# takkasila/practical_path_guiding_lab

Hardware: AMD Instinct MI355X
Metric: Msamples/s guided, veach-ajar 1920x1080 max_depth 13 (higher is better)
Workload: dtype f32; 1 GPU; veach-ajar 1920x1080, max_depth 13, 16 one-sample training passes (main.py:192, 218) per step in one batched launch (the whole film), guided iteration 6 (SD-tree trained by rendering iterations 0-5, 252 spp); full PathGuidingIntegrator.sample(): camera rays, NEE, BSDF/SD-tree MIS, record list, po...; spp_per_pass=16, passes_per_launch=16, steps_per_launch=1, kd_leaves=21429, quad_records=1675769, jump_bits=6, kd_grid_bits=6, bytes_jump_tables=1404370944, pixels_per_rank_min=2073600, pixels_per_rank_max=2073600

## Files before the change

### practical_path_guiding_lab_amd/csrc/pg_kernels_splat.hip

```cpp
#include "pg_descent.hpp"
#include "pg_kernels.hpp"
#include "pg_splat_dev.hpp"

namespace pg {

constexpr int kBlock = 256;
static_assert(kBlock == kStageThreads, "stage_kd_planes copies one plane per thread");

__device__ __forceinline__ void plan_record(const TreeView &t, const AccumView &a, const uint4 *s_kd, int store_nee,
                                            float x, float y, float z, float dx, float dy, float radiance,
                                            float wo_pdf, float nx, float ny, float nee_lum, SlotAdd &path,
                                            SlotAdd &nee, unsigned &kd_lv, unsigned &q_lv, unsigned &q_q, unsigned &bytes)
{
	const bool inside = inside_root(t, x, y, z);
	KdNode leaf;
	uint32_t lv;
	kd_descend_grid(t, reinterpret_cast<const float *>(s_kd), x, y, z, inside, leaf, lv);
	kd_lv += stat_levels(lv);
	bytes += stat_bytes(lv);
	const uint32_t tree = leaf.tree;
	const TreeHead head = load_head_s(t.head, tree);
	const JumpPre pre_p = jump_prefetch(t.jump, tree, dx, dy, in_unit_square(dx, dy));
	const JumpPre pre_n = jump_prefetch(t.jump, tree, nx, ny, store_nee != 0 && in_unit_square(nx, ny));
	const float w = wo_pdf > 0.0f ? radiance / wo_pdf : 0.0f;
// ... 121 lines not shown
	const bool single = t.n_rec == 0 && t.n_trees == 1;
	long long v[4] = {0, 0, 0, 0};
	unsigned kd_lv = 0, q_lv = 0, q_q = 0, did = 0, st_bytes = 0;
	for (uint64_t base = (uint64_t)blockIdx.x * kBlock; base < total; base += (uint64_t)gridDim.x * kBlock) {
		const uint64_t g = base + threadIdx.x;
		float radiance = 0.0f, nee_lum = 0.0f, wp = 0.0f;
		SlotAdd path = {nullptr, 0, 0, 0, 0}, nee = {nullptr, 0, 0, 0, 0};
		bool keep = false;
		if (g < total) keep = process_slot(g, S, num_rays, g / (uint64_t)max_depth, r.active[g] != 0, l_final, r, radiance, nee_lum, wp);
		if (keep) {
			plan_record(t, a, s_kd, store_nee, r.position[g], r.position[S + g], r.position[2 * S + g], r.direction[g],
			            r.direction[S + g], radiance, wp, r.direction_nee[g], r.direction_nee[S + g], nee_lum, path, nee,
			            kd_lv, q_lv, q_q, st_bytes);
			++did;
		}
		if (single) {
			if (path.ptr) { v[0] += path.w0; v[1] += path.w1; v[2] += path.w2; v[3] += path.w3; }
			if (nee.ptr) { v[0] += nee.w0; v[1] += nee.w1; v[2] += nee.w2; v[3] += nee.w3; }
		} else {
			coop_add(path, s_val, s_ptr);
			if (store_nee) coop_add(nee, s_val, s_ptr);
		}
	}
	if (single) {
		__syncthreads();
#pragma unroll
		for (int k = 0; k < 4; ++k) {
			const unsigned long long sw = wave_sum_s((unsigned long long)v[k]);
			if ((threadIdx.x & 63) == 0) s_val[(threadIdx.x >> 6) * 4 + k] = (long long)sw;
		}
		__syncthreads();
		if (threadIdx.x < 4) {
			unsigned long long tot = 0;
			for (int w = 0; w < kBlock / 64; ++w) tot += (unsigned long long)s_val[w * 4 + threadIdx.x];
			if (tot) atomicAdd(reinterpret_cast<unsigned long long *>(a.root_acc + threadIdx.x), tot);
		}
	}
	count_depths_s(dc, kd_lv, did, q_lv, q_q, st_bytes);
}

__global__ __launch_bounds__(kBlock) void k_splat_list(TreeView t, AccumView a, int store_nee, uint64_t num_rays,
                                                       int32_t max_depth, const float *__restrict__ l_final,
                                                       const uint4 *__restrict__ l_final_q, pg_list_records r,
                                                       const uint32_t *__restrict__ live_count)
{
	__shared__ long long s_val[kBlock * 4];
	__shared__ unsigned long long s_ptr[kBlock];
	const uint64_t S = num_rays * (uint64_t)max_depth;
	uint64_t total = num_rays;
	for (int b = 0; b + 1 < max_depth; ++b) total += live_count[b];
	if ((uint64_t)blockIdx.x * kBlock >= total) return;
	const bool single = t.n_rec == 0 && t.n_trees == 1;
	long long v[4] = {0, 0, 0, 0};
	for (uint64_t base = (uint64_t)blockIdx.x * kBlock; base < total; base += (uint64_t)gridDim.x * kBlock) {
		const uint64_t g = base + threadIdx.x;
		SlotAdd path = {nullptr, 0, 0, 0, 0}, nee = {nullptr, 0, 0, 0, 0};
		if (g < total) {
#define PG_LD(p) __builtin_nontemporal_load(p)
			const uint32_t ray = PG_LD(r.ray_of + g);
			if (ray != kNoRay) {
				float in[3], lf[3];
				if (l_final_q) {
					const uint4 q = l_final_q[ray];
					lf[0] = __uint_as_float(q.x); lf[1] = __uint_as_float(q.y); lf[2] = __uint_as_float(q.z);
				} else {
					lf[0] = l_final[ray]; lf[1] = l_final[num_rays + ray]; lf[2] = l_final[2 * num_rays + ray];
				}
#pragma unroll
				for (int ch = 0; ch < 3; ++ch) {
					float out = (lf[ch] - PG_LD(r.throughput_radiance + ch * S + g)) / PG_LD(r.throughput_bsdf + ch * S + g);
					if (out != out) out = 0.0f;
					float q = out / PG_LD(r.bsdf + ch * S + g);
					if (q != q) q = 0.0f;
					in[ch] = q;
				}
				float radiance = luminance(in[0], in[1], in[2]);
				if (radiance != radiance) radiance = 0.0f;
				const float nee_lum = PG_LD(r.nee_lum + g);
				const float wp = PG_LD(r.wo_pdf + g);
				const bool both_zero = (radiance == 0.0f) && (nee_lum == 0.0f);
				if (!both_zero && !(wp == 0.0f) && !(wp != wp)) {
					const uint2 sl = r.slot[g];
					const uint32_t tf = PG_LD(r.tree + g), tree = tf & 0x7fffffffu;
#undef PG_LD
					const bool inside = (tf >> 31) != 0u;
					const float w = wp > 0.0f ? radiance / wp : 0.0f;
					const float wn = wp > 0.0f ? nee_lum / wp : 0.0f;
					if (sl.x != kSlotNone) {
						const Limbs q = quantize_weight(w);
						path.ptr = sl.x == kSlotRoot ? a.root_acc + (size_t)kAccWords * tree : a.rec_acc + (size_t)kAccWords * sl.x;
						path.w0 = q.l0; path.w1 = q.l1; path.w2 = q.l2; path.w3 = inside ? 1 : 0;
					} else if (inside) {
						atomicAdd(a.leaf_count + tree, 1ull);
					}
					if (store_nee && sl.y != kSlotNone) {
						const Limbs q = quantize_weight(wn);
						nee.ptr = sl.y == kSlotRoot ? a.root_acc + (size_t)kAccWords * tree : a.rec_acc + (size_t)kAccWords * sl.y;
						nee.w0 = q.l0; nee.w1 = q.l1; nee.w2 = q.l2; nee.w3 = 0;
					}
				}
			}
		}
		if (single) {
			if (path.ptr) { v[0] += path.w0; v[1] += path.w1; v[2] += path.w2; v[3] += path.w3; }
			if (nee.ptr) { v[0] += nee.w0; v[1] += nee.w1; v[2] += nee.w2; v[3] += nee.w3; }
		} else {
			coop_add(path, s_val, s_ptr);
			if (store_nee) coop_add(nee, s_val, s_ptr);
		}
	}
	if (single) {
		__syncthreads();
#pragma unroll
		for (int k = 0; k < 4; ++k) {
			const unsigned long long sw = wave_sum_s((unsigned long long)v[k]);
			if ((threadIdx.x & 63) == 0) s_val[(threadIdx.x >> 6) * 4 + k] = (long long)sw;
		}
		__syncthreads();
		if (threadIdx.x < 4) {
			unsigned long long tot = 0;
			for (int w = 0; w < kBlock / 64; ++w) tot += (unsigned long long)s_val[w * 4 + threadIdx.x];
			if (tot) atomicAdd(reinterpret_cast<unsigned long long *>(a.root_acc + threadIdx.x), tot);
		}
	}
}

constexpr unsigned kSplatGroupsPerCu = 64;

static inline dim3 grid_for(uint64_t n) { return dim3((unsigned)((n + kBlock - 1) / kBlock)); }

void launch_splat(const TreeView &t, const AccumView &a, int store_nee, uint64_t m, const pg_records &rec,
                  const uint32_t *d_count, DepthCounters *dc, hipStream_t s)
{
	if (m == 0) return;
	hipLaunchKernelGGL(k_splat, grid_for(m), dim3(kBlock), 0, s, t, a, store_nee, m, rec.position,
	                   rec.direction, rec.radiance, rec.wo_pdf, rec.direction_nee, rec.radiance_nee_lum,
	                   d_count, dc);
}

void launch_process_records(uint64_t num_rays, int32_t max_depth, const float *l_final,
                            const pg_dense_records &rec, const pg_records_out &out, uint32_t *d_count,
                            hipStream_t s)
{
	const uint64_t S = num_rays * (uint64_t)max_depth;
	(void)hipMemsetAsync(d_count, 0, sizeof(uint32_t), s);
	if (S == 0) return;
	hipLaunchKernelGGL(k_process_records, grid_for(S), dim3(kBlock), 0, s, num_rays, max_depth, l_final, rec,
	                   out, d_count);
}

static dim3 strided_grid(uint64_t S)
{
	static int cus[64] = {0};
	int dev = 0;
	(void)hipGetDevice(&dev);
// ... 31 lines not shown
```

### practical_path_guiding_lab_amd/csrc/pg_render.hip

```cpp
#include "pg_render_dev.hpp"
#include "pg_scene_state.hpp"

namespace pg {


constexpr int kBounceStash = 17;
typedef __attribute__((address_space(3))) float LdsFloat;
template <bool kFirst, int kGeneral, bool kStash = false>
__device__ __forceinline__ bool bounce_lane(const RenderArgs &a, const uint4 *s_kd, const uint64_t lane,
                                            const uint64_t rec_slot, const uint32_t depth, LdsFloat *stash = nullptr)
{
	const uint64_t N = a.n_lanes;
	const int D = a.max_depth;
	const float f = a.frac;
	const Shapes &sh = a.shapes;
	Pcg32 rng;
	v3 ray_o, ray_d, thr, L, prev_p;
	float prev_bsdf_pdf;
	const bool prev_delta = kFirst;
	const float ior = 1.0f;
	static_assert(kGeneral < 2, "mesh scenes run the split pipeline of pg_render_wave.hip");
	if (kFirst) {
		const uint64_t pixel = global_pixel(a, lane / (uint64_t)a.spp);
		rng = lane_stream(a.seed, a.spp, a.batched, pixel, (uint32_t)(lane % (uint64_t)a.spp));
// ... 234 lines not shown
{
	__shared__ float s_planes[3 * kKdGridPlanes];
	const uint4 *s_kd = reinterpret_cast<const uint4 *>(s_planes);
	__shared__ uint32_t s_wave[kRBlock / 64];
	__shared__ uint32_t s_base;
	__shared__ float s_stash[kBounceStash][kRBlock];
	uint64_t tid;
	bool alive;
	if (!wave_entry<kFirst>(a, tid, alive)) return;
	if (a.guided || a.record) stage_kd_planes(s_planes, a.tree);
	const uint64_t lane = alive ? (kFirst ? tid : (uint64_t)a.order_in[tid]) : 0;
	const uint64_t rec_base = kFirst ? 0 : records_before(a);
	bool cont = false;
	if (alive) cont = bounce_lane<kFirst, kGeneral, true>(a, s_kd, lane, rec_base + tid, (uint32_t)a.bounce, (LdsFloat *)&s_stash[0][threadIdx.x]);
	if (a.last) return;
	const unsigned long long ballot = __ballot(cont);
	const unsigned wl = threadIdx.x & 63u, wv = threadIdx.x >> 6;
	if (wl == 0) s_wave[wv] = (uint32_t)__popcll(ballot);
	__syncthreads();
	if (threadIdx.x == 0) {
		uint32_t tot = 0;
		for (int w = 0; w < kRBlock / 64; ++w) tot += s_wave[w];
		s_base = tot ? atomicAdd(&a.live_count[a.bounce], tot) : 0u;
	}
	__syncthreads();
	if (cont) {
		uint32_t off = s_base + (uint32_t)__popcll(ballot & ((1ull << wl) - 1ull));
		for (unsigned w = 0; w < wv; ++w) off += s_wave[w];
		a.order_out[off] = (uint32_t)lane;
	}
}

template <int kGeneral>
__global__ __launch_bounds__(kRBlock) void k_bounce_tail(RenderArgs a)
{
	__shared__ float s_planes[3 * kKdGridPlanes];
	const uint4 *s_kd = reinterpret_cast<const uint4 *>(s_planes);
	const uint64_t tid = (uint64_t)blockIdx.x * kRBlock + threadIdx.x;
	const uint64_t live = (uint64_t)live_final(a, a.bounce - 1);
	if (live > kTailPaths || (uint64_t)blockIdx.x * kRBlock >= live) return;
	if (tail_took_over(a, a.bounce - 1)) return;
	if (a.guided || a.record) stage_kd_planes(s_planes, a.tree);
	bool alive = tid < live;
	const uint64_t lane = alive ? (uint64_t)a.order_in[tid] : 0;
	const uint64_t rec_base = records_before(a);
	const uint64_t tail_base = rec_base + live;
	uint64_t slot = rec_base + tid;
	for (int depth = a.bounce; depth < a.max_depth; ++depth) {
		if (alive) alive = bounce_lane<false, kGeneral>(a, s_kd, lane, slot, (uint32_t)depth);
		if (!tail_next_slot(a, depth, alive, tail_base, slot)) break;
	}
}

__global__ __launch_bounds__(kRBlock) void k_layout_L(const uint4 *__restrict__ Lq, float *__restrict__ L, uint64_t N)
{
	const uint64_t i = (uint64_t)blockIdx.x * kRBlock + threadIdx.x;
	if (i >= N) return;
	const uint4 q = Lq[i];
	L[i] = __uint_as_float(q.x); L[N + i] = __uint_as_float(q.y); L[2 * N + i] = __uint_as_float(q.z);
}

__global__ __launch_bounds__(kRBlock) void k_finish(RenderArgs a, uint8_t *__restrict__ valid_out,
                                                    float *__restrict__ sumL, float *__restrict__ sumL2)
{
	const uint64_t pix = (uint64_t)blockIdx.x * kRBlock + threadIdx.x;
	if (pix >= a.n_pixels) return;
	const uint64_t N = a.n_lanes, P = a.film_pixels;
	const uint64_t gpix = global_pixel(a, pix);
	const uint64_t first = pix * (uint64_t)a.spp;
	if (valid_out)
		for (int s = 0; s < a.spp; ++s) valid_out[first + s] = a.hit0[first + s];
	if (sumL && sumL2) {
		float s1[3], s2[3];
		for (int c = 0; c < 3; ++c) { s1[c] = sumL[c * P + gpix]; s2[c] = sumL2[c * P + gpix]; }
		for (int s = 0; s < a.spp; ++s)
			for (int c = 0; c < 3; ++c) {
				const float v = a.L[c * N + first + s];
				s1[c] = s1[c] + v;
				s2[c] = s2[c] + v * v;
			}
		for (int c = 0; c < 3; ++c) { sumL[c * P + gpix] = s1[c]; sumL2[c * P + gpix] = s2[c]; }
	}
}

__global__ __launch_bounds__(kRBlock) void k_math_eval(int which, uint64_t n, const float *__restrict__ x,
                                                       float *__restrict__ out)
{
	const uint64_t i = (uint64_t)blockIdx.x * kRBlock + threadIdx.x;
	if (i >= n) return;
	const float v = x[i];
	float r, c;
	switch (which) {
	case 0: r = exp_f32(v); break;
	case 1: r = log_f32(v); break;
	case 2: r = erf_f32(v); break;
	case 3: r = erfinv_f32(v); break;
	case 4: sincos_f32(v, r, c); break;
	default: sincos_f32(v, c, r); break;
	}
	out[i] = r;
}

__device__ __forceinline__ float tent1(float d)
{
	const float a = 1.0f - fabs_(d);
	return a > 0.0f ? a : 0.0f;
}

__device__ __forceinline__ float gauss1(float d)
{
	const float a = exp_f32(-2.0f * (d * d)) - exp_f32(-8.0f);
	return a > 0.0f ? a : 0.0f;
}

template <int kFilter, bool kBatched>
__global__ __launch_bounds__(kRBlock) void k_film(uint32_t seed, int spp, int W, int H,
                                                  const float *__restrict__ L, float *__restrict__ out,
                                                  uint32_t stripe_rows, uint32_t stripe_index, uint32_t stripe_count,
                                                  float *__restrict__ acc, float scale, int acc_set)
{
	constexpr int R = kFilter == 1 ? 2 : 1;
	const uint64_t npix = (uint64_t)W * (uint64_t)H, N = npix * (uint64_t)spp;
	const uint64_t o = (uint64_t)blockIdx.x * kRBlock + threadIdx.x;
	if (o >= npix) return;
	const int x = (int)(o % (uint64_t)W), y = (int)(o / (uint64_t)W);
	if (stripe_count > 1u && ((uint32_t)y / stripe_rows) % stripe_count != stripe_index) return;
	const float cx = (float)x + 0.5f, cy = (float)y + 0.5f;
	for (int img = 0; img < (kBatched ? spp : 1); ++img) {
		float a0 = 0.0f, a1 = 0.0f, a2 = 0.0f, wsum = 0.0f;
		for (int ny = y - R; ny <= y + R; ++ny)
			for (int nx = x - R; nx <= x + R; ++nx) {
				if (nx < 0 || ny < 0 || nx >= W || ny >= H) continue;
				const uint64_t pix = (uint64_t)ny * (uint64_t)W + (uint64_t)nx;
				for (int s = kBatched ? img : 0; s < (kBatched ? img + 1 : spp); ++s) {
					const uint64_t lane = pix * (uint64_t)spp + (uint64_t)s;
// ... 245 lines not shown
		                                     (ctx->filter_spatial ? "stochastic box" : "nearest") + ", directional " +
		                                     (ctx->filter_directional ? "box" : "nearest") + "); reset it to nearest / nearest, record through pg_splat / pg_process_and_splat, or set the scene with pg_render_record_geometry on");
	PG_HIP(ctx, hipSetDevice(ctx->device));
	const pg_camera &cam = ctx->render->scene.cam;
	const uint64_t film = (uint64_t)cam.width * (uint64_t)cam.height;
	if (prm->pixel_begin > film || prm->pixel_count > film - prm->pixel_begin)
		return fail(ctx, PG_ERR_INVALID, "pg_render_pass: pixel range outside the film");
	P = prm->pixel_count ? prm->pixel_count : film - prm->pixel_begin;
	if (prm->stripe_count > 1) {
		if (prm->stripe_rows == 0 || prm->stripe_index >= prm->stripe_count || prm->pixel_begin != 0)
			return fail(ctx, PG_ERR_INVALID, "pg_render_pass: bad stripe parameters");
		uint64_t rows = 0;
		for (uint64_t row = 0; row < (uint64_t)cam.height; ++row)
			rows += (row / prm->stripe_rows) % prm->stripe_count == prm->stripe_index;
		if (prm->pixel_count && prm->pixel_count != rows * (uint64_t)cam.width)
			return fail(ctx, PG_ERR_INVALID, "pg_render_pass: pixel_count does not match the stripes of this rank");
		P = rows * (uint64_t)cam.width;
	}
	if (P == 0) return PG_OK;
	if (P * (uint64_t)prm->spp * (uint64_t)ctx->max_depth > 0xffffffffull)
		return fail(ctx, PG_ERR_INVALID, "pg_render_pass: more than 2^32 record slots in one pass");
	if (prm->slot < 0 || prm->slot > 1) return fail(ctx, PG_ERR_INVALID, "pg_render_pass: slot must be 0 or 1");
	return PG_OK;
}

static RenderArgs pass_args(pg_context *ctx, const pg_pass_params *prm, PassBuf &b, uint64_t P, float *L_out)
{
	const pg_render_state *r = ctx->render;
	const int D = ctx->max_depth;
	RenderArgs a;
	a.tree = ctx->view();
	const SceneState &sc = r->scene;
	a.shapes.quads = sc.quads.p; a.shapes.spheres = sc.spheres.p; a.shapes.boxes = sc.boxes.p; a.shapes.tris = sc.tris.p;
	a.shapes.tri_normals = sc.have_tri_normals ? sc.tri_normals.p : nullptr;
	a.shapes.tri_uvs = sc.have_tri_uvs ? sc.tri_uvs.p : nullptr;
	a.shapes.textures = sc.textures.p; a.shapes.texels = sc.texels.p; a.shapes.srgb_lut = sc.srgb_lut.p;
	a.shapes.bvh = sc.bvh.p; a.shapes.n_bvh_nodes = sc.n_bvh_nodes;
	a.shapes.n_quads = sc.n_quads; a.shapes.n_spheres = sc.n_spheres; a.shapes.n_boxes = sc.n_boxes;
	a.mats = sc.mats.p; a.emitters = sc.emitters.p; a.n_emitters = sc.n_emitters; a.ior = r->ior.p;
	a.dir_lights.lights = sc.dir_lights.p;
	for (int c = 0; c < 4; ++c) a.dir_lights.bsphere[c] = sc.bsphere[c];
	a.cam = sc.cam;
	a.n_lanes = P * (uint64_t)prm->spp; a.n_pixels = P; a.pixel_begin = prm->pixel_begin;
	a.stripe_rows = prm->stripe_rows; a.stripe_index = prm->stripe_index; a.stripe_count = prm->stripe_count;
	a.film_pixels = (uint64_t)r->scene.cam.width * (uint64_t)r->scene.cam.height;
	a.spp = prm->spp; a.max_depth = D; a.rr_depth = prm->rr_depth; a.seed = prm->seed; a.batched = prm->batched ? 1 : 0;
	a.guided = ctx->iteration > 1 ? 1 : 0;
	a.record = ctx->is_final ? 0 : 1; a.store_nee = ctx->store_nee; a.frac = ctx->bsdf_fraction;
	a.dc = ctx->dc_on ? ctx->dc : nullptr;
	a.ph = ctx->ph_on ? ctx->ph_buf.p : nullptr;
	const bool wave = r->scene.general >= 2;
	a.fuse_guide = wave && r->stages < 2 && !(r->overlap & 1) ? 1 : 0;
	if (r->scene.geometry && a.record) a.fuse_guide = 0;
	a.ray_d = b.ray_d.p; a.thr = b.thr.p; a.L = L_out; a.prev_p = b.prev_p.p;
	a.prev_pdf = b.prev_pdf.p; a.prev_quad = b.prev_quad.p; a.hit0 = b.hit0.p;
	a.rng_state = b.rng_state.p; a.rng_inc = b.rng_inc.p; a.live_count = b.live_count.p;
	a.ray_of = b.ray_of.p; a.r_bsdf = b.r_bsdf.p; a.r_tb = b.r_tb.p;
	a.r_tr = b.r_tr.p; a.r_nee = b.r_nee.p; a.r_wp = b.r_wp.p;
	a.r_slot = b.r_slot.p; a.r_tree = b.r_tree.p;
	a.Lq = wave ? b.Lq.p : nullptr;
	a.ws = b.ws.p; a.bvh_ovf = b.bvh_ovf.p; a.shadow_list = b.shadow_list.p;
	a.cast_count = b.live_count.p + (D + 1);
	a.shadow_count = b.live_count.p + (D + 1) + 2 * D;
	a.st_in = nullptr; a.st_out = nullptr; a.inc_in = nullptr; a.inc_out = nullptr;
	a.sort_key = nullptr; a.perm = nullptr; a.carry_in = nullptr; a.carry_out = nullptr; a.n_sort = 0;
	return a;
}

static void quad_bounce(pg_render_state *r, const RenderArgs &a, int it, hipStream_t s)
{
	Timed t(r, s, Timer::Bounce);
	if (tail_checkpoint(it, a.max_depth)) {
		const dim3 tgrid((unsigned)((kTailPaths + kRBlock - 1) / kRBlock));
		if (r->scene.general == 1) hipLaunchKernelGGL((k_bounce_tail<1>), tgrid, dim3(kRBlock), 0, s, a);
		else hipLaunchKernelGGL((k_bounce_tail<0>), tgrid, dim3(kRBlock), 0, s, a);
	}
	const dim3 grid((unsigned)((a.n_lanes + kRBlock - 1) / kRBlock));
	if (r->scene.general == 1) {
		if (it == 0) hipLaunchKernelGGL((k_bounce<true, 1>), grid, dim3(kRBlock), 0, s, a);
		else hipLaunchKernelGGL((k_bounce<false, 1>), grid, dim3(kRBlock), 0, s, a);
	} else {
		if (it == 0) hipLaunchKernelGGL((k_bounce<true, 0>), grid, dim3(kRBlock), 0, s, a);
		else hipLaunchKernelGGL((k_bounce<false, 0>), grid, dim3(kRBlock), 0, s, a);
	}
}

static bool worth_sorting(const PassBuf &b, int bounce, int sort_until, uint64_t N)
{
	if (bounce < 1 || bounce >= sort_until) return false;
	return !b.live_known || (uint64_t)b.live_prev[bounce - 1] * kSortMinLiveDen >= N * kSortMinLiveNum;
}

static Timer timer_of(WaveStage stage)
{
	switch (stage) {
	case WaveStage::Trace: return Timer::Trace;
	case WaveStage::ShadeA: case WaveStage::Shade: return Timer::ShadeA;
	case WaveStage::Cast: return Timer::Shadow;
	case WaveStage::Guide: return Timer::Guide;
	case WaveStage::ShadeB: return Timer::ShadeB;
	case WaveStage::Tail: break;
	}
	return Timer::Tail;
}

static int wave_bounce(pg_context *ctx, PassBuf &b, RenderArgs &a, int it, int sort_until, hipStream_t s)
{
	pg_render_state *r = ctx->render;
	const uint64_t N = a.n_lanes;
	const unsigned blocks = (unsigned)((N + kRBlock - 1) / kRBlock);
	uint32_t *const geo = r->scene.geometry && a.record ? b.r_geo.p : nullptr;
	auto launch = [&](WaveStage stage, hipStream_t on, unsigned grid_blocks) {
		Timed t(r, on, timer_of(stage));
		launch_wave_stage(stage, r->scene.general, it == 0, a, grid_blocks, (unsigned)ctx->n_cus, on, geo);
	};
	a.st_in = b.st[it & 1].p; a.inc_in = b.inc[it & 1].p;
	a.st_out = b.st[(it + 1) & 1].p; a.inc_out = b.inc[(it + 1) & 1].p;
	const bool sorted = worth_sorting(b, it, sort_until, N);
	a.carry_in = sorted ? b.carry[it & 1].p : nullptr;
	a.sort_key = nullptr; a.perm = nullptr; a.carry_out = nullptr;
	if (tail_checkpoint(it, a.max_depth)) launch(WaveStage::Tail, s, (unsigned)((kTailPaths + kRBlock - 1) / kRBlock));
	a.sort_key = sorted ? b.sort_key.p : nullptr;
	a.carry_out = worth_sorting(b, it + 1, sort_until, N) ? b.carry[(it + 1) & 1].p : nullptr;
	const bool fork = (r->overlap & 1) && !sorted;
	if (fork && !b.side) {
		PG_HIP(ctx, hipStreamCreateWithFlags(&b.side, hipStreamNonBlocking));
		PG_HIP(ctx, hipEventCreateWithFlags(&b.ev_fork, hipEventDisableTiming));
		PG_HIP(ctx, hipEventCreateWithFlags(&b.ev_join, hipEventDisableTiming));
	}
	if (sorted) {
		const uint64_t n_sort = b.live_known ? (uint64_t)b.live_prev[it - 1] + (uint64_t)b.live_prev[it - 1] / 32 + 65536 : N;
		a.n_sort = (uint32_t)(n_sort < N ? n_sort : N);
		PG_HIP(ctx, hipMemsetAsync(b.sort_key.p, 0xff, (size_t)a.n_sort * sizeof(uint16_t), s));
	}
	launch(WaveStage::Trace, s, blocks);
	if (sorted) {
		Timed t(r, s, Timer::Sort);
		PG_HIP(ctx, sort_places16(b.sort_tmp.p, b.sort_tmp_bytes, b.sort_key.p, b.sort_key_out.p, b.sort_perm.p, a.n_sort,
		                            a.live_count + (it - 1), s));
		a.perm = b.sort_perm.p;
	}
	if (r->stages == 0 && !(r->overlap & 1) && !geo) {
		launch(WaveStage::Shade, s, blocks);
		return PG_OK;
	}
	launch(WaveStage::ShadeA, s, blocks);
	if (fork) {
		PG_HIP(ctx, hipEventRecord(b.ev_fork, s));
		PG_HIP(ctx, hipStreamWaitEvent(b.side, b.ev_fork, 0));
		launch(WaveStage::Guide, b.side, blocks);
		PG_HIP(ctx, hipEventRecord(b.ev_join, b.side));
	}
	launch(WaveStage::Cast, s, blocks);
	if (fork) PG_HIP(ctx, hipStreamWaitEvent(s, b.ev_join, 0));
	else if (!a.fuse_guide) launch(WaveStage::Guide, s, blocks);
	launch(WaveStage::ShadeB, s, blocks);
	return PG_OK;
}

static pg_list_geometry list_geometry(const PassBuf &b, uint64_t S)
{
	pg_list_geometry g;
	const float *f = reinterpret_cast<const float *>(b.r_geo.p);
	g.position = f + GEO_P * S; g.direction = f + GEO_WO * S; g.direction_nee = f + GEO_NEE * S;
	g.depth = b.r_geo.p + GEO_DEPTH * S;
	return g;
}

static pg_list_records list_records(const PassBuf &b)
{
	pg_list_records lr;
	lr.ray_of = b.ray_of.p; lr.bsdf = b.r_bsdf.p; lr.throughput_bsdf = b.r_tb.p; lr.throughput_radiance = b.r_tr.p;
	lr.nee_lum = b.r_nee.p; lr.wo_pdf = b.r_wp.p; lr.slot = b.r_slot.p; lr.tree = b.r_tree.p;
	return lr;
}

static int finish_pass(pg_context *ctx, int slot, const RenderArgs &a, uint8_t *valid_out, float *sumL, float *sumL2, hipStream_t s)
{
	pg_render_state *r = ctx->render;
	PassBuf &b = r->pb[slot];
	if (a.record) {
		Timed t(r, s, Timer::Splat);
		const pg_list_records lr = list_records(b);
		if (r->scene.geometry && ctx->filtered_launch())
			launch_splat_list_filtered(ctx->view(), ctx->f.accum_view(), ctx->filter_args(), ctx->store_nee, a.n_lanes, a.max_depth, a.Lq, lr,
			                           list_geometry(b, a.n_lanes * (uint64_t)a.max_depth), b.live_count.p, ctx->n_cus, s);
		else
			launch_splat_list(ctx->view(), ctx->f.accum_view(), ctx->store_nee, a.n_lanes, a.max_depth, a.L, a.Lq, lr, b.live_count.p, s);
		PG_HIP(ctx, hipGetLastError());
	}
	if (r->scene.general >= 2) {
		Timed t(r, s, Timer::Finish);
		hipLaunchKernelGGL(k_layout_L, dim3((unsigned)((a.n_lanes + kRBlock - 1) / kRBlock)), dim3(kRBlock), 0, s, b.Lq.p, a.L, a.n_lanes);
	}
	if (valid_out || sumL) {
		PassBuf &other = r->pb[1 - slot];
		if (sumL && other.finish_recorded) PG_HIP(ctx, hipStreamWaitEvent(s, other.ev_finish, 0));
		Timed t(r, s, Timer::Finish);
		hipLaunchKernelGGL(k_finish, dim3((unsigned)((a.n_pixels + kRBlock - 1) / kRBlock)), dim3(kRBlock), 0, s, a, valid_out,
		                   sumL, sumL2);
		PG_HIP(ctx, hipGetLastError());
		if (sumL) {
			if (!b.ev_finish) PG_HIP(ctx, hipEventCreateWithFlags(&b.ev_finish, hipEventDisableTiming));
			PG_HIP(ctx, hipEventRecord(b.ev_finish, s));
			b.finish_recorded = true;
		}
	}
	return PG_OK;
}

static void take_live_counts(PassBuf &b, uint64_t N, int D)
{
	if (b.live_pending && hipEventQuery(b.ev_live) == hipSuccess) {
		b.live_prev.assign(b.h_live, b.h_live + b.h_live_n);
		b.live_pending = false;
		b.live_known = true;
	}
	if (b.live_known && (b.live_prev_lanes != N || (int)b.live_prev.size() != D)) b.live_known = false;
}

static int send_live_counts(pg_context *ctx, PassBuf &b, uint64_t N, int D, hipStream_t s)
{
	if (!b.h_live || b.h_live_n != D) {
		if (b.h_live) (void)hipHostFree(b.h_live);
		b.h_live = nullptr;
		PG_HIP(ctx, hipHostMalloc((void **)&b.h_live, (size_t)D * sizeof(uint32_t)));
		b.h_live_n = D;
	}
	if (!b.ev_live) PG_HIP(ctx, hipEventCreateWithFlags(&b.ev_live, hipEventDisableTiming));
	if (!b.live_pending) {
		PG_HIP(ctx, hipMemcpyAsync(b.h_live, b.live_count.p, (size_t)D * sizeof(uint32_t), hipMemcpyDeviceToHost, s));
		PG_HIP(ctx, hipEventRecord(b.ev_live, s));
		b.live_pending = true;
		b.live_prev_lanes = N;
	}
	return PG_OK;
}

extern "C" {

int pg_render_pass(pg_context *ctx, const pg_pass_params *prm, float *L_out, uint8_t *valid_out, float *sumL,
                   float *sumL2, void *stream)
{
	uint64_t P = 0;
	int rc = check_pass(ctx, prm, L_out, sumL, sumL2, P);
	if (rc != PG_OK || P == 0) return rc;
	hipStream_t s = (hipStream_t)stream;
	pg_render_state *r = ctx->render;
	const int D = ctx->max_depth, slot = prm->slot;
	const uint64_t N = P * (uint64_t)prm->spp;
	PassBuf &b = r->pb[slot];
	r->last_slot = slot;
	if (sumL && (uint64_t)r->scene.cam.width * (uint64_t)r->scene.cam.height > ctx->num_rays)
// ... 243 lines not shown
```

### practical_path_guiding_lab_amd/csrc/pg_render_dev.hpp

```cpp
#pragma once

#include "pg_context.hpp"
#include "pg_descent.hpp"
#include "pg_kernels.hpp"
#include "pg_scene_layout.hpp"

#define PG_OUTLINE __forceinline__

namespace pg {

constexpr int kRBlock = 256;
static_assert(kRBlock == kStageThreads, "stage_kd_planes copies one plane per thread");
constexpr float kInvPiF = 0.31830988618379067154f;
constexpr float kRayEps = 1e-4f;
constexpr float kShadowEps = 1e-3f;

struct v3 {
	float x, y, z;
};
__device__ __forceinline__ v3 V(float x, float y, float z) { v3 r = {x, y, z}; return r; }
__device__ __forceinline__ v3 vadd(v3 a, v3 b) { return V(a.x + b.x, a.y + b.y, a.z + b.z); }
__device__ __forceinline__ v3 vsub(v3 a, v3 b) { return V(a.x - b.x, a.y - b.y, a.z - b.z); }
__device__ __forceinline__ v3 vmul(v3 a, v3 b) { return V(a.x * b.x, a.y * b.y, a.z * b.z); }
__device__ __forceinline__ v3 vscale(v3 a, float s) { return V(a.x * s, a.y * s, a.z * s); }
// ... 931 lines not shown
	}
	const v3 dir0 = vsub(pl, p);
	float mag = (1.0f + max3(V(fabs_(p.x), fabs_(p.y), fabs_(p.z)))) * kRayEps;
	if (dot3(n, dir0) < 0.0f) mag = -mag;
	const v3 so = vadd(p, vscale(n, mag));
	const float d2 = dot3(dir0, dir0), dist = __builtin_sqrtf(d2);
	ds_d = vdivs(dir0, dist);
	const float dp = dot3(ds_d, ln);
	float pdf = 0.0f;
	if (dp < 0.0f) pdf = is_sphere ? (dist == 0.0f ? 0.0f : pdf_cone) : d2 / (fabs_(dp) * area);
	if (!(pdf == pdf) || pdf == __builtin_huge_valf()) pdf = 0.0f;
	ds_pdf = pdf * inv_count;
	if (pdf > 0.0f) {
		const v3 sd = vsub(pl, so);
		const float sdist = __builtin_sqrtf(dot3(sd, sd));
		need_shadow = true;
		sh_o = so; sh_d = vdivs(sd, sdist); sh_tmax = sdist * (1.0f - kShadowEps);
		em_weight = vscale(vdivs(radiance, pdf), count);
	}
}

template <int kGeneral>
__device__ __forceinline__ void sample_emitter(const Shapes &sh, const DirLights &dls, const int32_t *__restrict__ emitters,
                                               int n_em, v3 p, v3 n, float e1, float e2, v3 &ds_d, float &ds_pdf,
                                               v3 &em_weight, bool &ds_delta)
{
	bool need_shadow;
	v3 sh_o, sh_d;
	float sh_tmax, th;
	sample_emitter_ray<kGeneral>(sh, dls, emitters, n_em, p, n, e1, e2, ds_d, ds_pdf, em_weight, ds_delta, need_shadow, sh_o, sh_d, sh_tmax);
	if (need_shadow && intersect<kGeneral, true>(sh, sh_o, sh_d, sh_tmax, th) >= 0) em_weight = V(0, 0, 0);
}

struct RenderArgs {
	TreeView tree;
	Shapes shapes;
	const float *mats;
	const int32_t *emitters;
	int n_emitters;
	DirLights dir_lights;
	float *ior;
	pg_camera cam;
	uint64_t n_lanes, n_pixels;
	uint64_t pixel_begin, film_pixels;
	uint32_t stripe_rows, stripe_index, stripe_count;
	int spp, max_depth, rr_depth, guided, record, store_nee;
	float frac;
	uint32_t seed;
	int batched;
	DepthCounters *dc;
	unsigned long long *ph;
	int bounce, last;
	int fuse_guide;
	const uint32_t *order_in;
	uint32_t *order_out;
	uint32_t *live_count;
	float *ray_d, *thr, *L, *prev_p, *prev_pdf;
	uint32_t *prev_quad;
	uint8_t *hit0;
	uint64_t *rng_state, *rng_inc;
	uint32_t *ray_of;
	float *r_bsdf, *r_tb, *r_tr, *r_nee, *r_wp;
	uint2 *r_slot;
	uint32_t *r_tree;
	const uint4 *st_in;
	uint4 *st_out;
	const uint64_t *inc_in;
	uint64_t *inc_out;
	uint16_t *sort_key;
	const uint32_t *perm;
	uint32_t n_sort;
	uint4 *carry_in, *carry_out;
	uint4 *Lq;
	uint32_t *ws;
	uint2 *bvh_ovf;
	uint32_t *cast_count, *shadow_count, *shadow_list;
};


constexpr uint32_t kTailPaths = 128u * 1024u;
__host__ __device__ constexpr bool tail_checkpoint(int bounce, int max_depth)
{
	return max_depth > 8 && bounce >= 4 && bounce + 1 < max_depth &&
	       (bounce < 8 || (bounce < 16 && bounce % 2 == 0) || bounce % 4 == 0);
}
typedef const __attribute__((address_space(4))) uint32_t *ConstU32Ptr;
__device__ __forceinline__ uint32_t live_final(const RenderArgs &a, int j)
{
	return reinterpret_cast<ConstU32Ptr>(reinterpret_cast<uintptr_t>(a.live_count))[j];
}
__device__ __forceinline__ uint64_t records_before(const RenderArgs &a)
{
	uint64_t r = a.n_lanes;
	for (int j = 0; j + 1 < a.bounce; ++j) r += live_final(a, j);
	return r;
}

__device__ __forceinline__ bool tail_took_over(const RenderArgs &a, int bounce)
{
	if (a.max_depth <= 8) return false;
	for (int c = 4; c <= bounce; ++c)
		if (tail_checkpoint(c, a.max_depth) && live_final(a, c - 1) <= kTailPaths) return true;
	return false;
}

template <bool kFirst>
// ... 51 lines not shown
```

### practical_path_guiding_lab_amd/csrc/pg_render_wave.hip

```cpp
#include "pg_render_dev.hpp"

namespace pg {

enum : int {
	WS_HIT_PRIM = 0, WS_HIT_T, WS_HIT_U, WS_HIT_V,
	WS_P, WS_NG = WS_P + 3,
	WS_FLAGS = WS_NG + 3,
	WS_U, WS_LE = WS_U + 10,
	WS_DS_D = WS_LE + 3, WS_DS_PDF = WS_DS_D + 3, WS_EM_W, WS_BV_EM = WS_EM_W + 3, WS_BP_EM = WS_BV_EM + 3,
	WS_SH_O, WS_SH_D = WS_SH_O + 3, WS_SH_T = WS_SH_D + 3,
	WS_WO_T, WS_ETA = WS_WO_T + 3,
	WS_RNG_LO, WS_RNG_HI,
	WS_OCC,
	WS_PDF_NEE, WS_PDF_TREE,
	WS_FWD, WS_FWD_THR = WS_FWD, WS_FWD_L = WS_FWD_THR + 4, WS_FWD_INC = WS_FWD_L + 4,
	WS_COUNT = WS_FWD_INC + 2
};

enum : uint32_t {
	F_VALID = 1u,
	F_ACTIVE_NEXT = 2u,
	F_ACTIVE_EM = 4u,
	F_NEED_SHADOW = 8u,
	F_DS_DELTA = 16u,
// ... 358 lines not shown
	const uint32_t m = ((spread5(c[0] >> 1) | (spread5(c[1] >> 1) << 1) | (spread5(c[2] >> 1) << 2)) << 1) | half;
	return m < 0xfffdu ? m : 0xfffdu;
}

constexpr int kBvhTopNodes = 48;
template <int kNodes>
__device__ __forceinline__ void stage_bvh_top(u32x4_t *s_top, const RenderArgs &a, BvhStack &stk)
{
	const uint32_t n = a.shapes.n_bvh_nodes < kNodes ? (uint32_t)a.shapes.n_bvh_nodes : (uint32_t)kNodes;
	constexpr int kLoads = (kNodes * kBvhNodeQuads + kRBlock - 1) / kRBlock;
	if (n) {
		u32x4_t v[kLoads];
#pragma unroll
		for (int k = 0; k < kLoads; ++k) {
			const uint32_t i = threadIdx.x + (uint32_t)k * kRBlock;
			v[k] = reinterpret_cast<const u32x4_t *>(a.shapes.bvh)[i < n * (uint32_t)kBvhNodeQuads ? i : 0u];
		}
#pragma unroll
		for (int k = 0; k < kLoads; ++k) {
			const uint32_t i = threadIdx.x + (uint32_t)k * kRBlock;
			if (i < n * (uint32_t)kBvhNodeQuads) s_top[i] = v[k];
		}
	}
	__syncthreads();
	stk.top = (const LdsQuad *)s_top;
	stk.n_top = n;
}

template <int kLevel, bool kFirst>
__global__ __launch_bounds__(kRBlock) void k_wave_trace(RenderArgs a)
{
	__shared__ uint2 s_stack[kLdsStack][kRBlock];
	uint64_t tid;
	bool alive;
	if (!wave_entry<kFirst>(a, tid, alive)) return;
	const bool want_cls = !kFirst && a.carry_in && a.guided && a.bounce + 1 < a.max_depth;
	uint4 q0 = make_uint4(0u, 0u, 0u, 0u), q1 = q0, q5 = q0;
	if (!kFirst) {
		const uint64_t it = alive ? tid : 0;
		const uint4 *p0 = a.carry_in ? st_rec(a.carry_in, it, PS_RAY_O) : a.st_in + it;
		const uint4 *p1 = a.carry_in ? st_rec(a.carry_in, it, PS_RAY_D) : a.st_in + a.n_lanes + it;
		const uint4 *p5 = a.carry_in ? st_rec(a.carry_in, it, PS_INC) : p0;
		q0 = *p0; q1 = *p1; q5 = *p5;
	}
	__shared__ u32x4_t s_top[kBvhTopNodes * kBvhNodeQuads];
	BvhStack stk = bvh_stack(&s_stack[0][threadIdx.x], a.bvh_ovf, (uint32_t)tid * (uint32_t)kOvfStack);
	stage_bvh_top<kBvhTopNodes>(s_top, a, stk);
	if (!alive) return;
	v3 ray_o, ray_d;
	int cls_ahead = -1;
	if (kFirst) {
		Pcg32 rng;
		camera_ray(a, tid, rng, ray_o, ray_d);
		const_cast<uint64_t *>(a.inc_in)[tid] = rng.inc;
		st_store(const_cast<uint4 *>(a.st_in), a, PS_RAY_O, tid, st_q(ray_o, (uint32_t)rng.state));
		st_store(const_cast<uint4 *>(a.st_in), a, PS_RAY_D, tid, st_q(ray_d, (uint32_t)(rng.state >> 32)));
	} else {
		ray_o = st_v3(q0);
		ray_d = st_v3(q1);
		if (want_cls && tid < (uint64_t)a.n_sort)
			cls_ahead = (int)lane_class_ahead(st_u64(q0.w, q1.w), st_u64(q5.x, q5.y), a.frac);
	}
	HitRec h;
	h.u = 0.0f; h.v = 0.0f;
	h.prim = intersect<kLevel, false>(a.shapes, ray_o, ray_d, __builtin_huge_valf(), h.t, stk, h.u, h.v);
	if (a.carry_in) {
		*st_rec(a.carry_in, tid, PS_HIT) = st_q_hit(h);
		if (tid < (uint64_t)a.n_sort) a.sort_key[tid] = (uint16_t)(h.prim >= 0 ? vertex_sort_key(a, vadd(ray_o, vscale(ray_d, h.t)), cls_ahead) : 0xfffeu);
		return;
	}
	wsputu(a, WS_HIT_PRIM, tid, (uint32_t)h.prim);
	wsput(a, WS_HIT_T, tid, h.t);
	wsput(a, WS_HIT_U, tid, h.u);
	wsput(a, WS_HIT_V, tid, h.v);
}

constexpr int kRefillIdle = 16;
constexpr uint32_t kCastChunk = 128;
template <int kLevel, bool kFirst>
__global__ __launch_bounds__(kRBlock) __attribute__((amdgpu_waves_per_eu(7))) void k_wave_cast(RenderArgs a)
{
	__shared__ uint2 s_stack[kLdsStack][kRBlock];
	if (!kFirst && tail_took_over(a, a.bounce)) return;
	const uint32_t total = kFirst ? (uint32_t)a.n_lanes : live_final(a, a.bounce - 1);
	const uint32_t gtid = blockIdx.x * kRBlock + threadIdx.x, n_static = gridDim.x * kRBlock;
	if (blockIdx.x * kRBlock >= total) return;
	const unsigned wl = threadIdx.x & 63u;
	const Shapes &sh = a.shapes;
	__shared__ u32x4_t s_top[kBvhTopNodes * kBvhNodeQuads];
	BvhStack stk = bvh_stack(&s_stack[0][threadIdx.x], a.bvh_ovf, gtid * (uint32_t)kOvfStack);
	stage_bvh_top<kBvhTopNodes>(s_top, a, stk);
	const int tri_base = sh.first_tri();
	BvhWalk w;
	w.next = kBvhNone; w.sp = 0; w.budget = 0; w.best = -1; w.bt = 0.0f; w.bu = 0.0f; w.bv = 0.0f;
	bool has = false, first_round = true;
	bool exhausted = n_static >= total;
	uint32_t pool_next = 0, pool_end = 0;
	const uint32_t n_waves = n_static / 64u;
	uint64_t chunk = gtid / 64u;
	uint32_t my = 0;
	for (;;) {
		const unsigned long long idle = __ballot(!has);
		const uint32_t n_idle = (uint32_t)__popcll(idle);
		if (first_round || (!exhausted && n_idle >= (uint32_t)kRefillIdle)) {
			uint32_t idx = 0xffffffffu;
			if (first_round) idx = gtid;
			else {
				if (pool_next == pool_end) {
					const uint64_t begin = (uint64_t)n_static + chunk * kCastChunk;
// ... 377 lines not shown
		__builtin_amdgcn_wave_barrier();
		__builtin_amdgcn_fence(__ATOMIC_ACQUIRE, "wavefront");
		cq0 = s_dyn[PS_RAY_O * kRBlock + threadIdx.x]; cq1 = s_dyn[PS_RAY_D * kRBlock + threadIdx.x]; cq2 = s_dyn[PS_THR * kRBlock + threadIdx.x];
		cq3 = s_dyn[PS_PREV * kRBlock + threadIdx.x]; cq4 = s_dyn[PS_L * kRBlock + threadIdx.x]; cq5 = s_dyn[PS_INC * kRBlock + threadIdx.x];
		cq6 = s_dyn[PS_HIT * kRBlock + threadIdx.x];
		__syncthreads();
	}
	uint2 *s_stack = reinterpret_cast<uint2 *>(s_dyn);
	u32x4_t *s_top = reinterpret_cast<u32x4_t *>(s_dyn) + kShadeStack * kRBlock / 2;
	BvhStack stk = bvh_stack(s_stack + threadIdx.x, a.bvh_ovf, (uint32_t)tid * (uint32_t)kOvfStack, kShadeStack);
#pragma unroll
	for (int k = 0; k < kPlaneLoads; ++k)
		if (a.tree.kd_grid != nullptr && threadIdx.x + k * kRBlock < 3u * kKdGridPlanes) s_planes[threadIdx.x + k * kRBlock] = pl_pre[k];
	if (a.tree.kd_grid != nullptr)
		for (uint32_t i = threadIdx.x + kPlaneLoads * kRBlock; i < 3u * kKdGridPlanes; i += kRBlock) s_planes[i] = a.tree.kd_planes[i];
#pragma unroll
	for (int k = 0; k < kTopLoads; ++k)
		if (threadIdx.x + k * kRBlock < n_top * 8u) s_top[threadIdx.x + k * kRBlock] = top_pre[k];
	__syncthreads();
	stk.top = (const LdsQuad *)s_top;
	stk.n_top = n_top;
	bool cont = false;
	v3 ray_o = V(0, 0, 0), ray_d = V(0, 0, 1), thr = V(1, 1, 1), L = V(0, 0, 0), p_here = V(0, 0, 0), prev_p = V(0, 0, 0);
	float ior = 1.0f, prev_pdf = 1.0f;
	bool delta = false, prev_delta = true;
	uint64_t lane = tid;
	Pcg32 rng;
	rng.state = 0; rng.inc = 1;
	uint64_t rec_base = 0;
	if (!kFirst) {
		rec_base = records_before(a);
		rec_base = (uint64_t)__builtin_amdgcn_readfirstlane((uint32_t)rec_base) |
		           ((uint64_t)__builtin_amdgcn_readfirstlane((uint32_t)(rec_base >> 32)) << 32);
	}
	if (alive) {
		HitRec h;
		const bool from_rec = !kFirst && a.perm != nullptr;
		uint32_t place = (uint32_t)tid;
		if (!coop && from_rec && tid < (uint64_t)a.n_sort) place = a.perm[tid];
		if (from_rec) {
			const uint4 *rec = st_rec(a.carry_in, place);
			uint4 q0, q1, q2, q3, q5, q6;
			if (coop) { q0 = cq0; q1 = cq1; q2 = cq2; q3 = cq3; q5 = cq5; q6 = cq6; }
			else { q0 = rec[PS_RAY_O]; q1 = rec[PS_RAY_D]; q2 = rec[PS_THR]; q3 = rec[PS_PREV]; q5 = rec[PS_INC]; q6 = rec[PS_HIT]; }
			rng.state = st_u64(q0.w, q1.w);
			rng.inc = st_u64(q5.x, q5.y);
			ray_o = st_v3(q0); ray_d = st_v3(q1);
			thr = st_v3(q2);
			{ const uint4 q4 = coop ? cq4 : rec[PS_L]; ior = st_ior(q2); L = st_v3(q4); lane = st_lane(q4); }
			prev_delta = st_delta(q2);
			prev_p = st_v3(q3);
			prev_pdf = st_wf(q3);
			h = st_hit(q6);
		} else {
			const uint4 q0 = st_load(a.st_in, a, PS_RAY_O, tid), q1 = st_load(a.st_in, a, PS_RAY_D, tid);
			rng.state = st_u64(q0.w, q1.w);
			rng.inc = a.inc_in[tid];
			ray_o = st_v3(q0); ray_d = st_v3(q1);
			if (!kFirst) {
				const uint4 q2 = st_load(a.st_in, a, PS_THR, tid), q3 = st_load(a.st_in, a, PS_PREV, tid);
				thr = st_v3(q2);
				{ const uint4 q4 = st_load(a.st_in, a, PS_L, tid); ior = st_ior(q2); L = st_v3(q4); lane = st_lane(q4); }
				prev_delta = st_delta(q2);
				prev_p = st_v3(q3);
				prev_pdf = st_wf(q3);
			}
			h = ws_hit(a, tid);
		}
		StageA A;
		PG_PHASE(0)
		stage_a1<kLevel>(a, rng, ray_o, ray_d, thr, prev_p, prev_pdf, prev_delta, h, (uint32_t)a.bounce, A);
		asm volatile("" : "+v"(A.flags), "+v"(A.wi.x), "+v"(A.wi.y), "+v"(A.wi.z), "+v"(A.p.x), "+v"(A.p.y), "+v"(A.p.z),
		                  "+v"(A.ng.x), "+v"(A.ng.y), "+v"(A.ng.z), "+v"(A.refl.x), "+v"(A.refl.y), "+v"(A.refl.z));
		asm volatile("" : "+v"(A.ds_d.x), "+v"(A.ds_d.y), "+v"(A.ds_d.z), "+v"(A.ds_pdf), "+v"(A.bp_em), "+v"(A.n.x), "+v"(A.n.y), "+v"(A.n.z));
		float *stash = reinterpret_cast<float *>(s_dyn) + (kShadeStack * kRBlock * 2 + kShadeTopNodes * 32) + threadIdx.x;
		stash[0 * kRBlock] = A.Le.x; stash[1 * kRBlock] = A.Le.y; stash[2 * kRBlock] = A.Le.z;
		stash[3 * kRBlock] = A.bv_em.x; stash[4 * kRBlock] = A.bv_em.y; stash[5 * kRBlock] = A.bv_em.z;
		stash[6 * kRBlock] = A.em_w.x; stash[7 * kRBlock] = A.em_w.y; stash[8 * kRBlock] = A.em_w.z;
		stash[9 * kRBlock] = thr.x; stash[10 * kRBlock] = thr.y; stash[11 * kRBlock] = thr.z;
		bool occluded = false;
		PG_PHASE(1)
		if (a.dc) {
			const unsigned long long m = __ballot((A.flags & F_NEED_SHADOW) != 0u);
			if ((threadIdx.x & 63u) == (unsigned)__builtin_ctzll(__ballot(1))) {
				atomicAdd(&a.dc->body_waves, 1ull);
				if (m) { atomicAdd(&a.dc->shadow_waves, 1ull); atomicAdd(&a.dc->shadow_lanes, (unsigned long long)__popcll(m)); }
			}
		}
		if (A.flags & F_NEED_SHADOW) {
			float th, bu, bv;
			occluded = intersect<kLevel, true, true>(a.shapes, A.sh_o, A.sh_d, A.sh_tmax, th, stk, bu, bv) >= 0;
		}
		PG_PHASE(2)
		asm volatile("" : "+v"(A.n.x), "+v"(A.n.y), "+v"(A.n.z), "+v"(A.mat));
		stage_a2<kLevel>(a, rng, A);
		asm volatile("" : "+v"(A.wo.x), "+v"(A.wo.y), "+v"(A.wo.z), "+v"(A.bsdf_w.x), "+v"(A.bsdf_w.y), "+v"(A.bsdf_w.z),
		                  "+v"(A.bsdf_pdf), "+v"(A.flags));
		if (kLevel >= 3) asm volatile("" : "+v"(A.eta));
		GuideOut g = guide_none(A.wo);
		PG_PHASE(3)
		if (guide_has_work(a, A.flags)) stage_guide(a, s_planes, rng, A.p, A.ds_d, (A.flags & F_SMP_TREE) ? V(0, 0, 0) : A.wo, A.flags, g);
		if (a.record && (A.flags & F_VALID)) store_slots(a, rec_base + tid, g);
		PG_PHASE(4)
		asm volatile("" : "+v"(A.n.x), "+v"(A.n.y), "+v"(A.n.z), "+v"(A.mat));
		A.Le = V(stash[0 * kRBlock], stash[1 * kRBlock], stash[2 * kRBlock]);
		A.bv_em = V(stash[3 * kRBlock], stash[4 * kRBlock], stash[5 * kRBlock]);
		A.em_w = V(stash[6 * kRBlock], stash[7 * kRBlock], stash[8 * kRBlock]);
		thr = V(stash[9 * kRBlock], stash[10 * kRBlock], stash[11 * kRBlock]);
		cont = stage_b<kLevel>(a, rng, thr, L, ior, A, g, occluded, lane, rec_base + tid, (uint32_t)a.bounce, ray_o, ray_d, prev_pdf, delta);
		p_here = A.p;
		if (kFirst) a.hit0[lane] = (A.flags & F_VALID) ? 1 : 0;
		if (!cont) end_path(a, lane, L);
		PG_PHASE(5)
	}
	append_survivors<kShadeStage>(a, cont, ray_o, ray_d, thr, ior, delta, p_here, prev_pdf, L, lane, rng, s_wave, s_base, s_oct, s_dyn);
	PG_PHASE(6)
#undef PG_PHASE
#if PG_SHADE_PHASES
	if (a.ph && (threadIdx.x & 63u) < 8u) {
// ... 161 lines not shown
```

Before: 730.3 Msamples/s.

## Prefetch splat ray ids, fuse L layout into finish, recompute first-bounce camera rays

The splat-list loop now software-prefetches the next iteration's ray index so its load overlaps the current iteration's work. The separate k_layout_L kernel is folded into a new k_finish_wave kernel that de-interleaves L, writes valid flags and accumulates per-pixel sums through shared memory, removing one launch and one pass over Lq. In the joint trace+shade path, the first bounce recomputes camera rays in shade instead of storing and reloading ray state, trading a little arithmetic for less global memory traffic. The sort-key memset before the trace is also dropped, which relies on the trace kernel writing every key it will read.

```diff
diff --git a/practical_path_guiding_lab_amd/csrc/pg_kernels_splat.hip b/practical_path_guiding_lab_amd/csrc/pg_kernels_splat.hip
--- a/practical_path_guiding_lab_amd/csrc/pg_kernels_splat.hip
+++ b/practical_path_guiding_lab_amd/csrc/pg_kernels_splat.hip
@@ -197,12 +197,16 @@
 	if ((uint64_t)blockIdx.x * kBlock >= total) return;
 	const bool single = t.n_rec == 0 && t.n_trees == 1;
 	long long v[4] = {0, 0, 0, 0};
-	for (uint64_t base = (uint64_t)blockIdx.x * kBlock; base < total; base += (uint64_t)gridDim.x * kBlock) {
+#define PG_LD(p) __builtin_nontemporal_load(p)
+	const uint64_t stride = (uint64_t)gridDim.x * kBlock;
+	const uint64_t g_first = (uint64_t)blockIdx.x * kBlock + threadIdx.x;
+	uint32_t ray_next = PG_LD(r.ray_of + (g_first < total ? g_first : 0));
+	if (g_first >= total) ray_next = kNoRay;
+	for (uint64_t base = (uint64_t)blockIdx.x * kBlock; base < total; base += stride) {
 		const uint64_t g = base + threadIdx.x;
 		SlotAdd path = {nullptr, 0, 0, 0, 0}, nee = {nullptr, 0, 0, 0, 0};
-		if (g < total) {
-#define PG_LD(p) __builtin_nontemporal_load(p)
-			const uint32_t ray = PG_LD(r.ray_of + g);
+		{
+			const uint32_t ray = ray_next;
 			if (ray != kNoRay) {
 				float in[3], lf[3];
 				if (l_final_q) {
@@ -227,7 +231,6 @@
 				if (!both_zero && !(wp == 0.0f) && !(wp != wp)) {
 					const uint2 sl = r.slot[g];
 					const uint32_t tf = PG_LD(r.tree + g), tree = tf & 0x7fffffffu;
-#undef PG_LD
 					const bool inside = (tf >> 31) != 0u;
 					const float w = wp > 0.0f ? radiance / wp : 0.0f;
 					const float wn = wp > 0.0f ? nee_lum / wp : 0.0f;
@@ -246,6 +249,9 @@
 				}
 			}
 		}
+		ray_next = PG_LD(r.ray_of + (g + stride < total ? g + stride : 0));
+		if (g + stride >= total) ray_next = kNoRay;
+#undef PG_LD
 		if (single) {
 			if (path.ptr) { v[0] += path.w0; v[1] += path.w1; v[2] += path.w2; v[3] += path.w3; }
 			if (nee.ptr) { v[0] += nee.w0; v[1] += nee.w1; v[2] += nee.w2; v[3] += nee.w3; }
diff --git a/practical_path_guiding_lab_amd/csrc/pg_render.hip b/practical_path_guiding_lab_amd/csrc/pg_render.hip
--- a/practical_path_guiding_lab_amd/csrc/pg_render.hip
+++ b/practical_path_guiding_lab_amd/csrc/pg_render.hip
@@ -310,14 +310,6 @@
 	}
 }
 
-__global__ __launch_bounds__(kRBlock) void k_layout_L(const uint4 *__restrict__ Lq, float *__restrict__ L, uint64_t N)
-{
-	const uint64_t i = (uint64_t)blockIdx.x * kRBlock + threadIdx.x;
-	if (i >= N) return;
-	const uint4 q = Lq[i];
-	L[i] = __uint_as_float(q.x); L[N + i] = __uint_as_float(q.y); L[2 * N + i] = __uint_as_float(q.z);
-}
-
 __global__ __launch_bounds__(kRBlock) void k_finish(RenderArgs a, uint8_t *__restrict__ valid_out,
                                                     float *__restrict__ sumL, float *__restrict__ sumL2)
 {
@@ -339,6 +331,41 @@
 			}
 		for (int c = 0; c < 3; ++c) { sumL[c * P + gpix] = s1[c]; sumL2[c * P + gpix] = s2[c]; }
 	}
+}
+
+__global__ __launch_bounds__(kRBlock) void k_finish_wave(RenderArgs a, uint8_t *__restrict__ valid_out, float *__restrict__ sumL,
+                                                         float *__restrict__ sumL2)
+{
+	__shared__ float s_L[3][kRBlock];
+	const uint64_t N = a.n_lanes, i = (uint64_t)blockIdx.x * kRBlock + threadIdx.x;
+	uint4 q = make_uint4(0u, 0u, 0u, 0u);
+	if (i < N) {
+		q = a.Lq[i];
+		a.L[i] = __uint_as_float(q.x); a.L[N + i] = __uint_as_float(q.y); a.L[2 * N + i] = __uint_as_float(q.z);
+		if (valid_out) valid_out[i] = a.hit0[i];
+	}
+	if (!(sumL && sumL2)) return;
+	s_L[0][threadIdx.x] = __uint_as_float(q.x); s_L[1][threadIdx.x] = __uint_as_float(q.y); s_L[2][threadIdx.x] = __uint_as_float(q.z);
+	__syncthreads();
+	if (i >= N || (uint32_t)i % (uint32_t)a.spp != 0u) return;
+	const uint64_t P = a.film_pixels;
+	const uint64_t gpix = global_pixel(a, (uint64_t)((uint32_t)i / (uint32_t)a.spp));
+	float s1[3], s2[3];
+	for (int c = 0; c < 3; ++c) { s1[c] = sumL[c * P + gpix]; s2[c] = sumL2[c * P + gpix]; }
+	for (int s = 0; s < a.spp; ++s) {
+		const uint32_t j = threadIdx.x + (uint32_t)s;
+		float v[3];
+		if (j < (uint32_t)kRBlock) { v[0] = s_L[0][j]; v[1] = s_L[1][j]; v[2] = s_L[2][j]; }
+		else {
+			const uint4 e = a.Lq[i + (uint64_t)s];
+			v[0] = __uint_as_float(e.x); v[1] = __uint_as_float(e.y); v[2] = __uint_as_float(e.z);
+		}
+		for (int c = 0; c < 3; ++c) {
+			s1[c] = s1[c] + v[c];
+			s2[c] = s2[c] + v[c] * v[c];
+		}
+	}
+	for (int c = 0; c < 3; ++c) { sumL[c * P + gpix] = s1[c]; sumL2[c * P + gpix] = s2[c]; }
 }
 
 __global__ __launch_bounds__(kRBlock) void k_math_eval(int which, uint64_t n, const float *__restrict__ x,
@@ -690,6 +717,7 @@
 	const bool wave = r->scene.general >= 2;
 	a.fuse_guide = wave && r->stages < 2 && !(r->overlap & 1) ? 1 : 0;
 	if (r->scene.geometry && a.record) a.fuse_guide = 0;
+	a.first_state_stored = 1;
 	a.ray_d = b.ray_d.p; a.thr = b.thr.p; a.L = L_out; a.prev_p = b.prev_p.p;
 	a.prev_pdf = b.prev_pdf.p; a.prev_quad = b.prev_quad.p; a.hit0 = b.hit0.p;
 	a.rng_state = b.rng_state.p; a.rng_inc = b.rng_inc.p; a.live_count = b.live_count.p;
@@ -754,6 +782,8 @@
 	};
 	a.st_in = b.st[it & 1].p; a.inc_in = b.inc[it & 1].p;
 	a.st_out = b.st[(it + 1) & 1].p; a.inc_out = b.inc[(it + 1) & 1].p;
+	const bool joint = r->stages == 0 && !(r->overlap & 1) && !geo;
+	a.first_state_stored = joint ? 0 : 1;
 	const bool sorted = worth_sorting(b, it, sort_until, N);
 	a.carry_in = sorted ? b.carry[it & 1].p : nullptr;
 	a.sort_key = nullptr; a.perm = nullptr; a.carry_out = nullptr;
@@ -769,7 +799,6 @@
 	if (sorted) {
 		const uint64_t n_sort = b.live_known ? (uint64_t)b.live_prev[it - 1] + (uint64_t)b.live_prev[it - 1] / 32 + 65536 : N;
 		a.n_sort = (uint32_t)(n_sort < N ? n_sort : N);
-		PG_HIP(ctx, hipMemsetAsync(b.sort_key.p, 0xff, (size_t)a.n_sort * sizeof(uint16_t), s));
 	}
 	launch(WaveStage::Trace, s, blocks);
 	if (sorted) {
@@ -778,7 +807,7 @@
 		                            a.live_count + (it - 1), s));
 		a.perm = b.sort_perm.p;
 	}
-	if (r->stages == 0 && !(r->overlap & 1) && !geo) {
+	if (joint) {
 		launch(WaveStage::Shade, s, blocks);
 		return PG_OK;
 	}
@@ -827,16 +856,17 @@
 			launch_splat_list(ctx->view(), ctx->f.accum_view(), ctx->store_nee, a.n_lanes, a.max_depth, a.L, a.Lq, lr, b.live_count.p, s);
 		PG_HIP(ctx, hipGetLastError());
 	}
-	if (r->scene.general >= 2) {
-		Timed t(r, s, Timer::Finish);
-		hipLaunchKernelGGL(k_layout_L, dim3((unsigned)((a.n_lanes + kRBlock - 1) / kRBlock)), dim3(kRBlock), 0, s, b.Lq.p, a.L, a.n_lanes);
-	}
-	if (valid_out || sumL) {
+	const bool wave = r->scene.general >= 2;
+	if (wave || valid_out || sumL) {
 		PassBuf &other = r->pb[1 - slot];
 		if (sumL && other.finish_recorded) PG_HIP(ctx, hipStreamWaitEvent(s, other.ev_finish, 0));
 		Timed t(r, s, Timer::Finish);
-		hipLaunchKernelGGL(k_finish, dim3((unsigned)((a.n_pixels + kRBlock - 1) / kRBlock)), dim3(kRBlock), 0, s, a, valid_out,
-		                   sumL, sumL2);
+		if (wave)
+			hipLaunchKernelGGL(k_finish_wave, dim3((unsigned)((a.n_lanes + kRBlock - 1) / kRBlock)), dim3(kRBlock), 0, s, a, valid_out,
+			                   sumL, sumL2);
+		else
+			hipLaunchKernelGGL(k_finish, dim3((unsigned)((a.n_pixels + kRBlock - 1) / kRBlock)), dim3(kRBlock), 0, s, a, valid_out,
+			                   sumL, sumL2);
 		PG_HIP(ctx, hipGetLastError());
 		if (sumL) {
 			if (!b.ev_finish) PG_HIP(ctx, hipEventCreateWithFlags(&b.ev_finish, hipEventDisableTiming));
diff --git a/practical_path_guiding_lab_amd/csrc/pg_render_dev.hpp b/practical_path_guiding_lab_amd/csrc/pg_render_dev.hpp
--- a/practical_path_guiding_lab_amd/csrc/pg_render_dev.hpp
+++ b/practical_path_guiding_lab_amd/csrc/pg_render_dev.hpp
@@ -1007,6 +1007,7 @@
 	unsigned long long *ph;
 	int bounce, last;
 	int fuse_guide;
+	int first_state_stored;
 	const uint32_t *order_in;
 	uint32_t *order_out;
 	uint32_t *live_count;
diff --git a/practical_path_guiding_lab_amd/csrc/pg_render_wave.hip b/practical_path_guiding_lab_amd/csrc/pg_render_wave.hip
--- a/practical_path_guiding_lab_amd/csrc/pg_render_wave.hip
+++ b/practical_path_guiding_lab_amd/csrc/pg_render_wave.hip
@@ -434,9 +434,11 @@
 	if (kFirst) {
 		Pcg32 rng;
 		camera_ray(a, tid, rng, ray_o, ray_d);
-		const_cast<uint64_t *>(a.inc_in)[tid] = rng.inc;
-		st_store(const_cast<uint4 *>(a.st_in), a, PS_RAY_O, tid, st_q(ray_o, (uint32_t)rng.state));
-		st_store(const_cast<uint4 *>(a.st_in), a, PS_RAY_D, tid, st_q(ray_d, (uint32_t)(rng.state >> 32)));
+		if (a.first_state_stored) {
+			const_cast<uint64_t *>(a.inc_in)[tid] = rng.inc;
+			st_store(const_cast<uint4 *>(a.st_in), a, PS_RAY_O, tid, st_q(ray_o, (uint32_t)rng.state));
+			st_store(const_cast<uint4 *>(a.st_in), a, PS_RAY_D, tid, st_q(ray_d, (uint32_t)(rng.state >> 32)));
+		}
 	} else {
 		ray_o = st_v3(q0);
 		ray_d = st_v3(q1);
@@ -920,19 +922,20 @@
 			prev_p = st_v3(q3);
 			prev_pdf = st_wf(q3);
 			h = st_hit(q6);
+		} else if (kFirst) {
+			camera_ray(a, tid, rng, ray_o, ray_d);
+			h = ws_hit(a, tid);
 		} else {
 			const uint4 q0 = st_load(a.st_in, a, PS_RAY_O, tid), q1 = st_load(a.st_in, a, PS_RAY_D, tid);
 			rng.state = st_u64(q0.w, q1.w);
 			rng.inc = a.inc_in[tid];
 			ray_o = st_v3(q0); ray_d = st_v3(q1);
-			if (!kFirst) {
-				const uint4 q2 = st_load(a.st_in, a, PS_THR, tid), q3 = st_load(a.st_in, a, PS_PREV, tid);
-				thr = st_v3(q2);
-				{ const uint4 q4 = st_load(a.st_in, a, PS_L, tid); ior = st_ior(q2); L = st_v3(q4); lane = st_lane(q4); }
-				prev_delta = st_delta(q2);
-				prev_p = st_v3(q3);
-				prev_pdf = st_wf(q3);
-			}
+			const uint4 q2 = st_load(a.st_in, a, PS_THR, tid), q3 = st_load(a.st_in, a, PS_PREV, tid);
+			thr = st_v3(q2);
+			{ const uint4 q4 = st_load(a.st_in, a, PS_L, tid); ior = st_ior(q2); L = st_v3(q4); lane = st_lane(q4); }
+			prev_delta = st_delta(q2);
+			prev_p = st_v3(q3);
+			prev_pdf = st_wf(q3);
 			h = ws_hit(a, tid);
 		}
 		StageA A;
```

New measurement: 735.7 Msamples/s (median of 6 runs). Within noise of the previous version (+0.7%).
